# mwhoffman/pygp

Hardware: AMD Instinct MI355X
Metric: ExactGP log-lik+grad evals/sec at N=16384 D=8 SE-ARD fp64 (higher is better)
Workload: dtype f64; 1 GPU; ExactGP SE-ARD fp64 loglik+grad, N=16384 D=8 (metric config); batched-theta path: 6 independent thetas per GPU per step through gpx_loglik_batch, X/y resident in HBM; safe_mode=False, safe_mode_switches=0, launch=one process, C ABI only (no torch)

## Files before the change

### include/gpx.h

```cpp
#ifndef GPX_H
#define GPX_H

#include <stdint.h>

#ifdef __cplusplus
extern "C" {
#endif

#define GPX_VERSION 100
#define GPX_MAX_DIM 32
#define GPX_MAX_PARTS 8
#define GPX_MAX_HYPER (GPX_MAX_PARTS * (GPX_MAX_DIM + 2))

enum gpx_kind {
    GPX_SE = 1,
    GPX_MATERN1 = 2,
    GPX_MATERN3 = 3,
    GPX_MATERN5 = 4,
    GPX_PERIODIC = 5,
    GPX_SUM = 6,
    GPX_RQ = 7,
    GPX_PRODUCT = 8
};

// ... 83 lines not shown
int gpx_ep_update(gpx_t *h, const gpx_kspec *k, double mean, double tol, int max_iter,
                  double damping, int *iters, int *info);
int gpx_ep_loglik(gpx_t *h, double *lZ, double *dlZ);
int gpx_ep_posterior(gpx_t *h, const double *Xs, int64_t m, double *mu, double *s2);
int gpx_ep_posterior_full(gpx_t *h, const double *Xs, int64_t m, double *mu, double *Sigma);
int gpx_ep_get_sites(gpx_t *h, int64_t n, double *tau, double *nu, double *mu, double *s2);
int gpx_ep_timings(gpx_t *h, double *ms);
int gpx_exact_get_factor(gpx_t *h, int64_t n, double *R, double *a);
int gpx_loglik_batch(gpx_t *h, const gpx_kspec *k, const double *thetas,
                     int64_t B, int want_grad, double *lZ, double *dlZ,
                     int *info);
int gpx_batch_plan(gpx_t *h, int64_t B, int want_grad, int *plan);
int gpx_loglik_batch_multi(const gpx_kspec *k, const double *thetas, int64_t B,
                           const double *X, const double *y, int64_t n, int64_t d,
                           int want_grad, int ndev, double *lZ, double *dlZ, int *info);
int gpx_posterior_batch_multi(const gpx_kspec *k, const double *thetas, int64_t B,
                              const double *X, const double *y, int64_t n, int64_t d,
                              const double *Xs, int64_t m, int want_grad, int ndev, double *mu,
                              double *s2, double *dmu, double *ds2, int *info);
int gpx_multi_enable_timing(int ndev, int on);
int gpx_multi_batch_info(int ndev, int64_t B_per_dev, int want_grad, double *dense_ms,
                         int64_t *members, int *plans);
void gpx_batch_partition(int64_t B, int world, int rank, int64_t *lo, int64_t *hi);
int64_t gpx_multi_slot(int64_t B, int ndev);
int gpx_multi_comm_size(void);
int gpx_multi_pack(const double *rows, int64_t cnt, int width, int64_t slot, double *pack);
int gpx_multi_scatter(const double *gathered, int64_t B, int ndev, int width, double *out);
int gpx_posterior_batch(gpx_t *h, const gpx_kspec *k, const double *thetas, int64_t B,
                        const double *Xs, int64_t m, double *mu, double *s2, double *dmu,
                        double *ds2, int *info);

#define GPX_SPARSE_MAX_P 4096
enum gpx_sparse_method { GPX_FITC = 1, GPX_DTC = 2, GPX_VFE = 3 };
int gpx_sparse_update(gpx_t *h, const gpx_kspec *k, int method, const double *U, int64_t p,
                      double log_sn, double mean, int *info);
int gpx_sparse_append(gpx_t *h, const double *Xnew, const double *ynew, int64_t m, int *info);
int gpx_sparse_loglik(gpx_t *h, double *lZ, double *dlZ);
int gpx_sparse_posterior(gpx_t *h, const double *Xs, int64_t m, double *mu, double *s2,
                         double *dmu, double *ds2);
int gpx_sparse_posterior_full(gpx_t *h, const double *Xs, int64_t m, double *mu, double *Sigma);
int gpx_sparse_get_state(gpx_t *h, double *F1, double *F2, double *v);
int gpx_sparse_timings(gpx_t *h, double *ms);
int gpx_sparse_loglik_pseudo(gpx_t *h, double *lZ, double *dlZ, double *dU);
int gpx_sparse_pseudo_timing(gpx_t *h, double *ms);

int gpx_select_pivots(gpx_t *h, const gpx_kspec *k, const double *X, int64_t n, int64_t d,
                      int64_t p, double tol, int64_t *idx, double *piv, double *trace,
                      int64_t *count);
int gpx_select_timing(gpx_t *h, double *ms);

#define GPX_NTIMERS 11
int gpx_enable_timing(gpx_t *h, int on);
int gpx_get_timings(gpx_t *h, double *ms, int n);
int gpx_batch_timings(gpx_t *h, double *dense_ms, int64_t *members);
const char *gpx_timing_name(int i);

int gpx_la_gemm(gpx_t *h, int ta, int tb, int64_t M, int64_t N, int64_t K,
                double alpha, const double *A, int64_t lda, const double *B,
                int64_t ldb, double beta, double *C, int64_t ldc);
typedef struct gpx_gemm_ex_args {
    int64_t ta, tb, M, N, K, lda, ldb, ldc;
    double alpha, beta;
    int64_t flags, tile, waves, order, swizzle, use_lists, kshift, beta0_from;
    int64_t batch, strideA, strideB, strideC, strideC2;
    int64_t kchunk, nsplit, mstrideA, mstrideB, mstrideC;
    int64_t offA, offB, offC, offC2;
    int64_t b_is_c;
} gpx_gemm_ex_args;
int gpx_la_gemm_ex(gpx_t *h, const gpx_gemm_ex_args *a, const double *A, int64_t nA,
                   const double *B, int64_t nB, double *C, int64_t nC, double *C2,
                   int64_t nC2);
int gpx_la_potrf(gpx_t *h, const double *A, int64_t n, double *R, double *Rinv,
                 double *Ainv, int *info);
int gpx_la_gemm_bench(gpx_t *h, int ta, int tb, int64_t n, int reps, double *ms);
int gpx_la_gemm_bench_ex(gpx_t *h, int ta, int tb, int64_t n, int flags, int order,
                         int swizzle, int tile, int waves, int same_ab, int reps,
                         double *ms);
int gpx_la_gemm_bench_mnk(gpx_t *h, int ta, int tb, int64_t M, int64_t N, int64_t K, int flags,
                          double beta, int tile, int reps, double *ms);
int gpx_la_potrf_bench(gpx_t *h, int64_t n, int with_inverse, int reps,
                       double *ms);

int gpx_panel_graph_check(int T, int workers, int stream, int *ntasks);
int gpx_panel_grid_check(int nmem, int ncu, int *nspwg, int *workers);
int gpx_panel_graph_check_wide(int T, int E, int workers, int *ntasks);
int gpx_panel_graph_check_rhs(int T, int workers, int *ntasks);
int gpx_panel_graph_check_full(int T, int workers, int *ntasks);
int gpx_panel_solo_check(int T, int aug, int full, int value_only, int *ntasks);
int gpx_sweep_check(int T, int aug);
int gpx_sweep_check_lite(int T, int aug, int depth);

#ifdef __cplusplus
}
#endif
#endif
```

### pygp_amd/_lib.py

```python

import ctypes as C
import os
import threading

import numpy as np

__all__ = ['lib', 'Handle', 'default_handle', 'kspec_of', 'GpxError', 'device_count',
           'loglik_batch_multi', 'batch_partition',
           'KIND_SE', 'KIND_MATERN', 'KIND_PERIODIC', 'KIND_SUM', 'KIND_RQ', 'KIND_PRODUCT',
           'F64',
           'F32']

_HERE = os.path.dirname(os.path.abspath(__file__))
_LIBPATH = os.path.join(_HERE, 'libgpx.so')

KIND_SE = 1
KIND_MATERN = {1: 2, 3: 3, 5: 4}
KIND_PERIODIC = 5
KIND_SUM = 6
KIND_RQ = 7
KIND_PRODUCT = 8
F64, F32 = 0, 1
NTIMERS = 11

# ... 53 lines not shown
    'gpx_exact_eval': (C.c_int, [_vp, C.POINTER(_KSpec), C.c_double, C.c_double,
                                 C.c_int, _dp, _vp, _ip]),
    'gpx_exact_posterior': (C.c_int, [_vp, _vp, _i64, _vp, _vp]),
    'gpx_exact_posterior_grad': (C.c_int, [_vp, _vp, _i64, _vp, _vp, _vp, _vp]),
    'gpx_exact_posterior_full': (C.c_int, [_vp, _vp, _i64, _vp, _vp]),
    'gpx_kernel_gradx': (C.c_int, [_vp, C.POINTER(_KSpec), _vp, _i64, _vp, _i64, _i64,
                                   C.c_int, _vp]),
    'gpx_kernel_gradxy': (C.c_int, [_vp, C.POINTER(_KSpec), _vp, _i64, _vp, _i64, _i64, _vp]),
    'gpx_exact_posterior_gradient': (C.c_int, [_vp, _vp, _i64, _vp, _vp]),
    'gpx_gradobs_set_data': (C.c_int, [_vp, _vp, _i64, _vp, _vp, _i64, _vp, _i64]),
    'gpx_gradobs_update': (C.c_int, [_vp, C.POINTER(_KSpec), C.c_double, C.c_double,
                                     C.c_double, _ip]),
    'gpx_gradobs_loglik': (C.c_int, [_vp, _dp]),
    'gpx_gradobs_posterior': (C.c_int, [_vp, _vp, _i64, _vp, _vp]),
    'gpx_gradobs_posterior_full': (C.c_int, [_vp, _vp, _i64, _vp, _vp]),
    'gpx_kernel_matvec': (C.c_int, [_vp, C.POINTER(_KSpec), _vp, _i64, _i64, _vp, _i64, _vp]),
    'gpx_laplace_set_data': (C.c_int, [_vp, _vp, _i64, _i64, _vp]),
    'gpx_laplace_update': (C.c_int, [_vp, C.POINTER(_KSpec), C.c_int, C.c_double, C.c_double,
                                     C.c_int, C.c_int, _ip, _ip]),
    'gpx_laplace_loglik': (C.c_int, [_vp, _dp, _vp]),
    'gpx_laplace_posterior': (C.c_int, [_vp, _vp, _i64, _vp, _vp]),
    'gpx_laplace_posterior_full': (C.c_int, [_vp, _vp, _i64, _vp, _vp]),
    'gpx_laplace_get_mode': (C.c_int, [_vp, _i64, _vp, _vp]),
    'gpx_laplace_timings': (C.c_int, [_vp, _vp]),
    'gpx_ep_update': (C.c_int, [_vp, C.POINTER(_KSpec), C.c_double, C.c_double, C.c_int,
                                C.c_double, _ip, _ip]),
    'gpx_ep_loglik': (C.c_int, [_vp, _dp, _vp]),
    'gpx_ep_posterior': (C.c_int, [_vp, _vp, _i64, _vp, _vp]),
    'gpx_ep_posterior_full': (C.c_int, [_vp, _vp, _i64, _vp, _vp]),
    'gpx_ep_get_sites': (C.c_int, [_vp, _i64, _vp, _vp, _vp, _vp]),
    'gpx_ep_timings': (C.c_int, [_vp, _vp]),
    'gpx_mo_set_data': (C.c_int, [_vp, _vp, _i64, _vp, _i64, _i64]),
    'gpx_mo_update': (C.c_int, [_vp, C.POINTER(_KSpec), C.c_double, C.c_double, _ip]),
    'gpx_mo_loglik': (C.c_int, [_vp, _dp, _vp]),
    'gpx_mo_posterior': (C.c_int, [_vp, _vp, _i64, _vp, _vp]),
    'gpx_mo_posterior_full': (C.c_int, [_vp, _vp, _i64, _vp, _vp]),
    'gpx_icm_set_data': (C.c_int, [_vp, _vp, _i64, _i64, _vp, _vp, _i64]),
    'gpx_icm_update': (C.c_int, [_vp, C.POINTER(_KSpec), _vp, _vp, _vp, _ip]),
    'gpx_icm_loglik': (C.c_int, [_vp, _dp, _vp]),
    'gpx_icm_posterior': (C.c_int, [_vp, _vp, _vp, _i64, _vp, _vp]),
    'gpx_icm_posterior_full': (C.c_int, [_vp, _vp, _vp, _i64, _vp, _vp]),
    'gpx_exact_get_factor': (C.c_int, [_vp, _i64, _vp, _vp]),
    'gpx_sparse_update': (C.c_int, [_vp, C.POINTER(_KSpec), C.c_int, _vp, _i64, C.c_double,
                                    C.c_double, _ip]),
    'gpx_sparse_append': (C.c_int, [_vp, _vp, _vp, _i64, _ip]),
    'gpx_sparse_loglik': (C.c_int, [_vp, _vp, _vp]),
    'gpx_sparse_posterior': (C.c_int, [_vp, _vp, _i64, _vp, _vp, _vp, _vp]),
    'gpx_sparse_posterior_full': (C.c_int, [_vp, _vp, _i64, _vp, _vp]),
    'gpx_sparse_get_state': (C.c_int, [_vp, _vp, _vp, _vp]),
    'gpx_sparse_timings': (C.c_int, [_vp, _vp]),
    'gpx_sparse_loglik_pseudo': (C.c_int, [_vp, _vp, _vp, _vp]),
    'gpx_sparse_pseudo_timing': (C.c_int, [_vp, _vp]),
    'gpx_select_pivots': (C.c_int, [_vp, C.POINTER(_KSpec), _vp, _i64, _i64, _i64, C.c_double,
                                    _vp, _vp, _vp, C.POINTER(_i64)]),
    'gpx_select_timing': (C.c_int, [_vp, _vp]),
    'gpx_loglik_batch': (C.c_int, [_vp, C.POINTER(_KSpec), _vp, _i64, C.c_int,
                                   _vp, _vp, _vp]),
    'gpx_batch_plan': (C.c_int, [_vp, _i64, C.c_int, _ip]),
    'gpx_loglik_batch_multi': (C.c_int, [C.POINTER(_KSpec), _vp, _i64, _vp, _vp, _i64, _i64,
                                         C.c_int, C.c_int, _vp, _vp, _vp]),
    'gpx_posterior_batch_multi': (C.c_int, [C.POINTER(_KSpec), _vp, _i64, _vp, _vp, _i64, _i64,
                                            _vp, _i64, C.c_int, C.c_int, _vp, _vp, _vp, _vp,
                                            _vp]),
    'gpx_batch_partition': (None, [_i64, C.c_int, C.c_int, C.POINTER(_i64),
                                   C.POINTER(_i64)]),
    'gpx_multi_slot': (_i64, [_i64, C.c_int]),
    'gpx_multi_comm_size': (C.c_int, []),
    'gpx_multi_pack': (C.c_int, [_vp, _i64, C.c_int, _i64, _vp]),
    'gpx_multi_scatter': (C.c_int, [_vp, _i64, C.c_int, C.c_int, _vp]),
    'gpx_posterior_batch': (C.c_int, [_vp, C.POINTER(_KSpec), _vp, _i64, _vp, _i64, _vp,
                                      _vp, _vp, _vp, _vp]),
    'gpx_enable_timing': (C.c_int, [_vp, C.c_int]),
    'gpx_get_timings': (C.c_int, [_vp, _vp, C.c_int]),
    'gpx_batch_timings': (C.c_int, [_vp, _dp, C.POINTER(_i64)]),
    'gpx_timing_name': (C.c_char_p, [C.c_int]),
    'gpx_la_gemm': (C.c_int, [_vp, C.c_int, C.c_int, _i64, _i64, _i64,
                              C.c_double, _vp, _i64, _vp, _i64, C.c_double, _vp,
                              _i64]),
    'gpx_set_safe_mode': (C.c_int, [_vp, C.c_int]),
    'gpx_get_safe_mode': (C.c_int, [_vp, _ip]),
    'gpx_multi_enable_timing': (C.c_int, [C.c_int, C.c_int]),
    'gpx_multi_batch_info': (C.c_int, [C.c_int, _i64, C.c_int, _dp, C.POINTER(_i64), _ip]),
    'gpx_panel_grid_check': (C.c_int, [C.c_int, C.c_int, _ip, _ip]),
    'gpx_la_gemm_ex': (C.c_int, [_vp, _vp, _vp, _i64, _vp, _i64, _vp, _i64, _vp, _i64]),
    'gpx_la_potrf': (C.c_int, [_vp, _vp, _i64, _vp, _vp, _vp, _ip]),
    'gpx_la_gemm_bench': (C.c_int, [_vp, C.c_int, C.c_int, _i64, C.c_int, _dp]),
    'gpx_la_gemm_bench_ex': (C.c_int, [_vp, C.c_int, C.c_int, _i64, C.c_int, C.c_int,
                                       C.c_int, C.c_int, C.c_int, C.c_int, C.c_int,
                                       _dp]),
    'gpx_la_gemm_bench_mnk': (C.c_int, [_vp, C.c_int, C.c_int, _i64, _i64, _i64, C.c_int,
                                        C.c_double, C.c_int, C.c_int, _dp]),
    'gpx_la_potrf_bench': (C.c_int, [_vp, _i64, C.c_int, C.c_int, _dp]),
    'gpx_panel_graph_check': (C.c_int, [C.c_int, C.c_int, C.c_int, C.POINTER(C.c_int)]),
    'gpx_panel_graph_check_wide': (C.c_int, [C.c_int, C.c_int, C.c_int, C.POINTER(C.c_int)]),
    'gpx_panel_graph_check_rhs': (C.c_int, [C.c_int, C.c_int, C.POINTER(C.c_int)]),
    'gpx_panel_graph_check_full': (C.c_int, [C.c_int, C.c_int, C.POINTER(C.c_int)]),
    'gpx_panel_solo_check': (C.c_int, [C.c_int, C.c_int, C.c_int, C.c_int, C.POINTER(C.c_int)]),
    'gpx_sweep_check': (C.c_int, [C.c_int, C.c_int]),
    'gpx_sweep_check_lite': (C.c_int, [C.c_int, C.c_int, C.c_int]),
}

_lib = None
_lock = threading.RLock()


def lib():
    global _lib
    if _lib is None:
        with _lock:
            if _lib is None:
                if not os.path.exists(_LIBPATH):
                    raise GpxError(
                        'pygp_amd/libgpx.so is missing: build it with '
                        '`python -m pygp_amd.build` (there is no CPU fallback)')
                L = C.CDLL(_LIBPATH)
                for name, (res, args) in SIGNATURES.items():
                    f = getattr(L, name)
                    f.restype, f.argtypes = res, args
                _lib = L
    return _lib


def _ptr(a):
    return None if a is None else a.ctypes.data_as(_vp)


def _f64(a, ndim=None):
    a = np.ascontiguousarray(a, dtype=np.float64)
    if ndim is not None and a.ndim != ndim:
        raise ValueError('expected a %d-d array' % ndim)
    return a


def _pair(X1, X2, dtype=np.float64):
    X1 = np.ascontiguousarray(X1, dtype=dtype)
    if X1.ndim != 2:
        raise ValueError('expected a 2-d array')
    n1, d = X1.shape
    if X2 is None:
        return X1, n1, None, n1, d
    X2 = np.ascontiguousarray(X2, dtype=dtype)
    if X2.ndim != 2 or X2.shape[1] != d:
        raise ValueError('X1 and X2 have different dimensions')
    return X1, n1, X2, X2.shape[0], d


def check(code):
    if code == 0:
        return
    msg = lib().gpx_last_error().decode('utf-8', 'replace')
    if code > 0:
        raise np.linalg.LinAlgError(
            '%d-th leading minor of the array is not positive definite' % code)
    raise GpxError(msg or 'libgpx error %d' % code)


class KSpecHolder(object):

    def __init__(self, kind, iso, ndim, hyper=None, parts=()):
        self.parts = list(parts)
        self.hyper = None if hyper is None else _f64(np.atleast_1d(hyper))
        self.c = _KSpec()
        self.c.kind, self.c.iso, self.c.ndim = kind, int(bool(iso)), int(ndim)
        if self.parts:
            self.arr = (_KSpec * len(self.parts))(*[p.c for p in self.parts])
            self.c.nparts = len(self.parts)
# ... 599 lines not shown
    B, nth = thetas.shape
    if nth != spec.c.nhyper + 2:
        raise ValueError('thetas must have %d columns' % (spec.c.nhyper + 2))
    if (X is None) != (y is None):
        raise ValueError('pass both X and y, or neither')
    n = d = 0
    if X is not None:
        X, y = _f64(X, 2), _f64(y, 1)
        if X.shape[0] != y.shape[0]:
            raise ValueError('X and y disagree')
        n, d = X.shape
    lZ = np.empty(B)
    dlZ = np.empty((B, nth)) if grad else None
    info = np.zeros(B, dtype=np.int32)
    check(lib().gpx_loglik_batch_multi(spec.ref(), _ptr(thetas), B, _ptr(X), _ptr(y), n, d,
                                       int(grad), int(ndev), _ptr(lZ), _ptr(dlZ),
                                       _ptr(info)))
    return (lZ, dlZ) if grad else lZ


def posterior_batch_multi(spec, thetas, Xs, X=None, y=None, grad=False, ndev=1, token=None):
    return _multi_call(lambda X_, y_: _posterior_batch_multi(spec, thetas, Xs, X_, y_, grad, ndev),
                       X, y, token, ndev)


def _posterior_batch_multi(spec, thetas, Xs, X, y, grad, ndev):
    thetas = _f64(thetas, 2)
    B, nth = thetas.shape
    if nth != spec.c.nhyper + 2:
        raise ValueError('thetas must have %d columns' % (spec.c.nhyper + 2))
    if (X is None) != (y is None):
        raise ValueError('pass both X and y, or neither')
    Xs = _f64(Xs, 2)
    m, d = Xs.shape
    n = 0
    if X is not None:
        X, y = _f64(X, 2), _f64(y, 1)
        if X.shape[0] != y.shape[0] or X.shape[1] != d:
            raise ValueError('X, y and Xs disagree')
        n = X.shape[0]
    mu, s2 = np.empty((B, m)), np.empty((B, m))
    dmu = np.empty((B, m, d)) if grad else None
    ds2 = np.empty((B, m, d)) if grad else None
    info = np.zeros(B, dtype=np.int32)
    check(lib().gpx_posterior_batch_multi(spec.ref(), _ptr(thetas), B, _ptr(X), _ptr(y), n,
                                          d if X is not None else 0, _ptr(Xs), m, int(grad),
                                          int(ndev), _ptr(mu), _ptr(s2), _ptr(dmu), _ptr(ds2),
                                          _ptr(info)))
    return (mu, s2, dmu, ds2) if grad else (mu, s2)


def batch_partition(B, world, rank):
    lo, hi = _i64(0), _i64(0)
    lib().gpx_batch_partition(B, world, rank, C.byref(lo), C.byref(hi))
    return lo.value, hi.value


def multi_comm_size():
    return int(lib().gpx_multi_comm_size())


def multi_enable_timing(ndev, on=True):
    check(lib().gpx_multi_enable_timing(int(ndev), int(bool(on))))


def multi_batch_info(ndev, B_per_dev, grad=False):
    ms = (C.c_double * ndev)()
    mem = (_i64 * ndev)()
    plans = (C.c_int * (4 * ndev))()
    check(lib().gpx_multi_batch_info(int(ndev), int(B_per_dev), int(grad), ms, mem, plans))
    return [{'device': i, 'dense_ms': float(ms[i]), 'members': int(mem[i]),
             'arrangement': ('contexts', 'groups/panel', 'groups/lockstep', 'groups/solo')[plans[4 * i]],
             'members_per_group': int(plans[4 * i + 1]),
             'groups_in_flight': int(plans[4 * i + 2]),
             'safe_mode': bool(plans[4 * i + 3])} for i in range(ndev)]


def panel_grid_check(nmem, ncu=256):
    sp, wk = C.c_int(0), C.c_int(0)
    check(lib().gpx_panel_grid_check(int(nmem), int(ncu), C.byref(sp), C.byref(wk)))
    return sp.value, wk.value


def multi_pack(rows, slot):
    rows = np.ascontiguousarray(rows, dtype=np.float64)
    cnt, width = rows.shape
    pack = np.empty((int(slot), width))
    check(lib().gpx_multi_pack(_ptr(rows) if cnt else None, cnt, width, int(slot), _ptr(pack)))
    return pack


def multi_scatter(gathered, B, ndev, width):
    gathered = np.ascontiguousarray(gathered, dtype=np.float64)
    out = np.full((int(B), int(width)), np.nan)
    check(lib().gpx_multi_scatter(_ptr(gathered) if B else None, int(B), int(ndev), int(width),
                                  _ptr(out) if B else None))
    return out


def sweep_check(T, aug=False):
    check(lib().gpx_sweep_check(int(T), int(bool(aug))))


def panel_solo_check(T, aug=False, full=False, value_only=False):
    n = C.c_int(0)
    check(lib().gpx_panel_solo_check(int(T), int(bool(aug)), int(bool(full)), int(bool(value_only)),
                                     C.byref(n)))
    return n.value


def sweep_check_lite(T, aug=False, depth=-1):
    check(lib().gpx_sweep_check_lite(int(T), int(bool(aug)), int(depth)))


def panel_graph_check_rhs(T, workers=64):
    n = C.c_int(0)
    check(lib().gpx_panel_graph_check_rhs(int(T), int(workers), C.byref(n)))
    return n.value


def panel_graph_check_full(T, workers=64):
    n = C.c_int(0)
    check(lib().gpx_panel_graph_check_full(int(T), int(workers), C.byref(n)))
    return n.value


def panel_graph_check(T, workers=64, stream=True, extra=0):
    n = C.c_int(0)
    if extra:
        check(lib().gpx_panel_graph_check_wide(int(T), int(extra), int(workers), C.byref(n)))
    else:
        check(lib().gpx_panel_graph_check(int(T), int(workers), int(bool(stream)), C.byref(n)))
    return n.value


_default = None


def default_handle():
    global _default
    if _default is None:
        with _lock:
            if _default is None:
                _default = Handle()
    return _default
```

### pygp_amd/csrc/chol.hip

```cpp

#include "gpx_internal.h"

#define LB GPX_TILE

#include <algorithm>
#include <vector>

__global__ __launch_bounds__(256) void copy_block_kernel(const double *__restrict__ src,
                                                         double *__restrict__ dst, int ld,
                                                         int rows, int cols, long long stride)
{
    src += (long long)blockIdx.z * stride;
    dst += (long long)blockIdx.z * stride;
    const int c2 = blockIdx.x * 256 + threadIdx.x;
    if (2 * c2 >= cols) return;
    for (int r = blockIdx.y; r < rows; r += gridDim.y)
        reinterpret_cast<double2 *>(dst + (size_t)r * ld)[c2] =
            reinterpret_cast<const double2 *>(src + (size_t)r * ld)[c2];
}

static int copy_block(hipStream_t s, const double *src, double *dst, int ld, int rows,
                      int cols, int batch = 1, long long stride = 0)
{
    dim3 grid((cols / 2 + 255) / 256, rows < 1024 ? rows : 1024, batch);
// ... 415 lines not shown
    hipEvent_t *G = w.events + 2 * GPX_MAX_BLOCKS;
    hipEvent_t *TD = w.events + 3 * GPX_MAX_BLOCKS;
    bool lead = false;
    if (ahead) {
        GPX_EV(hipEventRecord(D[0], s));
        const bool wide0 = nb > 1 && wide_ok(w, bl.len(0), bl.len(1), 1);
        lead = w.lead && w.lead_rows >= (wide0 ? bl.off(2) : bl.len(0));
        GPX_EV(hipStreamWaitEvent(crit, lead ? w.lead : D[0], 0));
        GPX_EV(hipStreamWaitEvent(bulk, D[0], 0));
        if (aux != bulk) GPX_EV(hipStreamWaitEvent(aux, D[0], 0));
    }
    for (int k = 0; k < nb; ++k) {
        const int ok = bl.off(k), nk = bl.len(k);
        if (ahead && k > 0) GPX_EV(hipStreamWaitEvent(crit, D[k], 0));
        const bool wide = k + 1 < nb && wide_ok(w, nk, bl.len(k + 1), 1);
        if (wide)
            GPX_TRY(gpx_panel(crit, w, ok, nk, bl.len(k + 1), w.gate_total[0], w.gate_total[1]));
        else
            GPX_TRY(potrf_rec(crit, w, ok, nk, true));
        if (ahead) {
            GPX_EV(hipEventRecord(F[k], crit));
            GPX_EV(hipStreamWaitEvent(bulk, F[k], 0));
            if (lead && k == 0) GPX_EV(hipStreamWaitEvent(crit, D[0], 0));
        }
        if (fast && k + 1 < nb) {
            const int o1 = bl.off(k + 1), n1 = bl.len(k + 1), rest = w.np - o1;
            const size_t okk = (size_t)ok * ld + ok, ok1 = (size_t)ok * ld + o1;
            const size_t o11 = (size_t)o1 * ld + o1;
            if (!wide) {
                if (k >= 1) GPX_EV(hipStreamWaitEvent(crit, G[k - 1], 0));
                {
                    GemmArgs g = mk(w.W + okk, ld, w.Kinv + ok1, ld, w.A + ok1, ld, nk, n1, nk,
                                    1.0, 0.0, GEMM_KHI_M);
                    g.order = gpx_env().ord_r12;
                    GPX_TRY(gpx_gemm(crit, 1, 0, g));
                }
                if (k >= 1) GPX_EV(hipStreamWaitEvent(crit, TD[k - 1], 0));
                GPX_TRY(syrk_upper(crit, w.A + ok1, ld, w.A + o11, ld, n1, nk, w.Kinv + o11));
            }
            GPX_EV(hipEventRecord(D[k + 1], crit));
            if (rest > n1) {
                GemmArgs g = mk(w.W + okk, ld, w.Kinv + ok1 + n1, ld, w.A + ok1 + n1, ld, nk,
                                rest - n1, nk, 1.0, 0.0, GEMM_KHI_M);
                g.order = gpx_env().ord_r12;
                GPX_TRY(gpx_gemm(bulk, 1, 0, g));
            }
            GPX_EV(hipStreamWaitEvent(bulk, D[k + 1], 0));
            if (k + 2 < nb) {
                const int o2 = bl.off(k + 2), n2 = bl.len(k + 2), rest2 = w.np - o2;
                const size_t ok2 = (size_t)ok * ld + o2, o12 = (size_t)o1 * ld + o2,
                             o22 = (size_t)o2 * ld + o2;
                {
                    GemmArgs g = mk(w.A + ok1, ld, w.A + ok2, ld, w.Kinv + o12, ld, n1, rest2,
                                    nk, -1.0, 1.0, 0);
                    GPX_TRY(gpx_gemm(bulk, 1, 0, g));
                }
                GPX_TRY(gate_bump(bulk, w, 0));
                GPX_EV(hipEventRecord(G[k], bulk));
                GPX_TRY(syrk_upper(bulk, w.A + ok2, ld, w.A + o22, ld, n2, nk, w.Kinv + o22));
                GPX_TRY(gate_bump(bulk, w, 1));
                GPX_EV(hipEventRecord(TD[k], bulk));
                if (k + 3 < nb) {
                    const int o3 = bl.off(k + 3), rest3 = w.np - o3;
                    const size_t ok3 = (size_t)ok * ld + o3, o23 = (size_t)o2 * ld + o3,
                                 o33 = (size_t)o3 * ld + o3;
                    GemmArgs g = mk(w.A + ok2, ld, w.A + ok3, ld, w.Kinv + o23, ld, n2, rest3, nk,
                                    -1.0, 1.0, 0);
                    GPX_TRY(gpx_gemm(bulk, 1, 0, g));
                    GPX_TRY(syrk_upper(bulk, w.A + ok3, ld, w.A + o33, ld, rest3, nk,
                                       w.Kinv + o33));
                }
            }
        } else if (k + 1 < nb) {
            const int o1 = bl.off(k + 1), n1 = bl.len(k + 1), rest = w.np - o1;
            const size_t okk = (size_t)ok * ld + ok, ok1 = (size_t)ok * ld + o1;
            const int skip = wide ? n1 : 0;
            if (rest > skip) {
                GemmArgs g = mk(w.W + okk, ld, w.Kinv + ok1 + skip, ld, w.A + ok1 + skip, ld, nk,
                                rest - skip, nk, 1.0, 0.0, GEMM_KHI_M);
                g.order = gpx_env().ord_r12;
                GPX_TRY(gpx_gemm(bulk, 1, 0, g));
            }
            const size_t o11 = (size_t)o1 * ld + o1;
            if (!wide)
                GPX_TRY(syrk_upper(bulk, w.A + ok1, ld, w.A + o11, ld, n1, nk, w.Kinv + o11));
            if (ahead) GPX_EV(hipEventRecord(D[k + 1], bulk));
            if (k + 2 < nb) {
                const int o2 = bl.off(k + 2), rest2 = w.np - o2;
                const size_t ok2 = (size_t)ok * ld + o2, o12 = (size_t)o1 * ld + o2,
                             o22 = (size_t)o2 * ld + o2;
                {
                    GemmArgs g = mk(w.A + ok1, ld, w.A + ok2, ld, w.Kinv + o12, ld, n1, rest2,
                                    nk, -1.0, 1.0, 0);
                    GPX_TRY(gpx_gemm(bulk, 1, 0, g));
                }
                GPX_TRY(gate_bump(bulk, w, 0));
                GPX_TRY(syrk_upper(bulk, w.A + ok2, ld, w.A + o22, ld, rest2, nk, w.Kinv + o22));
                GPX_TRY(gate_bump(bulk, w, 1));
            }
        }
        if (mode != GPX_POTRF_R)
            GPX_TRY(inverse_column(aux, w, bl, k, mode == GPX_POTRF_KINV,
                                   defer && k == nb - 1 ? evW : nullptr,
                                   ahead && aux != bulk && k > 0 ? D[k] : nullptr,
                                   ahead && aux != bulk ? F[k] : nullptr));
    }
    if (ahead) {
        GPX_EV(hipEventRecord(evJoin, bulk));
        GPX_EV(hipStreamWaitEvent(s, evJoin, 0));
        if (aux != bulk) {
            GPX_EV(hipEventRecord(evAux, aux));
            GPX_EV(hipStreamWaitEvent(s, defer ? evW : evAux, 0));
        }
    }
    return 0;
}

int gpx_potrf_join(hipStream_t s, const DenseWs &w)
{
    if (w.defer_kinv && w.events && w.aux)
        GPX_EV(hipStreamWaitEvent(s, w.events[4 * GPX_MAX_BLOCKS + 1], 0));
    return 0;
}

hipEvent_t gpx_potrf_lead_event(const DenseWs &w)
{
    return w.events ? w.events[4 * GPX_MAX_BLOCKS + 3] : nullptr;
}

int gpx_trtri(hipStream_t s, const DenseWs &w)
{
    const BatchScope batch_scope(w);
    const Blocks bl(w.np);
    return trtri_blocks(s, w, bl, 0, bl.count);
}

int gpx_trsm_rt(hipStream_t s, const DenseWs &w, double *B, double *T, int ldb, int m,
                long long pstride)
{
    const BatchScope batch_scope(w);
    const Blocks bl(w.np);
    const int ld = w.ld;
    const int nb = w.batch > 1 ? w.batch : 1;
    auto panel = [&](GemmArgs g, bool a_panel) {
        if (nb > 1) {
            if (a_panel) g.strideA = pstride;
            g.strideB = pstride;
            g.strideC = pstride;
        }
        return g;
    };
    for (int k = 0; k < bl.count; ++k) {
        const int ok = bl.off(k), nk = bl.len(k);
        const size_t okk = (size_t)ok * ld + ok;
        double *Bk = B + (size_t)ok * ldb, *Tk = T + (size_t)ok * ldb;
        if (nk == LB) {
            GemmArgs g = mk(w.W + okk, ld, Bk, ldb, Bk, ldb, LB, m, LB, 1.0, 0.0, 0);
            g.tile = 128;
            GPX_TRY(gpx_gemm(s, 1, 0, panel(g, false)));
        } else {
            GPX_TRY(copy_block(s, Bk, Tk, ldb, nk, m, nb, pstride));
            GemmArgs g = mk(w.W + okk, ld, Tk, ldb, Bk, ldb, nk, m, nk, 1.0, 0.0, GEMM_KHI_M);
            g.order = 1;
            GPX_TRY(gpx_gemm(s, 1, 0, panel(g, false)));
        }
        const int o1 = bl.off(k + 1), rest = w.np - o1;
        if (rest > 0)
            GPX_TRY(gpx_gemm(s, 1, 0,
                             panel(mk(w.A + (size_t)ok * ld + o1, ld, Bk, ldb, B + (size_t)o1 * ldb,
                                      ldb, rest, m, nk, -1.0, 1.0, 0), false)));
    }
    return 0;
}

int gpx_lauum(hipStream_t s, const DenseWs &w)
{
    const BatchScope batch_scope(w);
    const int n = w.np, ld = w.ld;
    GemmArgs g = mk(w.W, ld, w.W, ld, w.Kinv, ld, n, n, n, 1.0, 0.0,
                    GEMM_UPPER_ONLY | GEMM_KLO_M | GEMM_KLO_N |
// ... 12 lines not shown
```

### pygp_amd/csrc/gpx_env.h

```cpp
#pragma once

#include <cstdlib>
#include <cstring>
#include <vector>

#define GPX_ENV_TABLE(X)                                                        \
        \
    X(int, nb0, "GPX_NB0", 0)                                                   \
    X(int, nb, "GPX_NB", 0)                                                     \
    X(const char *, blocks_text, "GPX_BLOCKS", nullptr)                         \
    X(int, split_last, "GPX_SPLIT_LAST", 0)                                     \
    X(int, lookahead, "GPX_LOOKAHEAD", 1)                                       \
    X(int, fastchain, "GPX_FASTCHAIN", 1)                                       \
    X(int, aux, "GPX_AUX", 1)                                                   \
    X(int, lead_build, "GPX_LEAD_BUILD", 1)                                     \
    X(int, defer_kinv, "GPX_DEFER_KINV", 1)                                     \
    X(int, invcol_early, "GPX_INVCOL_EARLY", -1)                                \
    X(int, overlap_nosplit, "GPX_OVERLAP_NOSPLIT", 1)                           \
    X(int, grad_whole, "GPX_GRAD_WHOLE", 4096)                                  \
    X(int, grad_full_w, "GPX_GRAD_FULL_W", 4096)                                \
       \
    X(int, swizzle, "GPX_SWIZZLE", 0)                                           \
    X(int, tile_lists, "GPX_TILE_LISTS", 1)                                     \
    X(int, ord_t, "GPX_ORD_T", 2)                                               \
    X(int, ord_r12, "GPX_ORD_R12", 1)                                           \
    X(int, ord_lauum, "GPX_ORD_LAUUM", 0)                                       \
    X(int, krev, "GPX_KREV", 0)                                                 \
    X(int, krev_invcol, "GPX_KREV_INVCOL", 0)                                   \
    X(int, tile_xcd, "GPX_TILE_XCD", -1)                                        \
    X(int, gemm_big, "GPX_GEMM_BIG", 0)                                         \
    X(int, gemm_small, "GPX_GEMM_SMALL", 0)                                     \
    X(int, gemm_small_below, "GPX_GEMM_SMALL_BELOW", 0)                         \
    X(int, gemm_nobalance, "GPX_GEMM_NOBALANCE", 0)                             \
    X(int, gemm_nosplit, "GPX_GEMM_NOSPLIT", 0)                                 \
    X(int, gemm_pipe, "GPX_GEMM_PIPE", 1)                                       \
    X(const char *, gemm_log, "GPX_GEMM_LOG", nullptr)                          \
    X(int, ldpad, "GPX_LDPAD", 32)                                              \
    X(int, bench_ldpad, "GPX_BENCH_LDPAD", 0)                                   \
                                           \
    X(int, panel, "GPX_PANEL", -1)                                              \
    X(int, panel_stream, "GPX_PANEL_STREAM", 1)                                 \
    X(int, panel_serial, "GPX_PANEL_SERIAL", 1)                                 \
    X(int, panel_strict, "GPX_PANEL_STRICT", 0)                                 \
    X(int, panel_debug, "GPX_PANEL_DEBUG", 0)                                   \
    X(int, panel_timeout_ms, "GPX_PANEL_TIMEOUT_MS", 2000)                      \
    X(int, panel_timeout_us, "GPX_PANEL_TIMEOUT_US", 0)                         \
    X(int, panel_wg, "GPX_PANEL_WG", -1)                                        \
    X(int, panel_wg_wide, "GPX_PANEL_WG_WIDE", -1)                              \
    X(int, panel_wg_whole, "GPX_PANEL_WG_WHOLE", -1)                            \
    X(int, panel_nspine, "GPX_PANEL_NSPINE", -1)                                \
    X(int, panel_mspine, "GPX_PANEL_MSPINE", -1)                                \
    X(int, panel_mwg, "GPX_PANEL_MWG", -1)                                      \
    X(int, panel_split, "GPX_PANEL_SPLIT", 1)                                   \
    X(int, panel_fold, "GPX_PANEL_FOLD", 1)                                     \
    X(int, panel_kbatch, "GPX_PANEL_KBATCH", -1)                                \
    X(int, panel_i128, "GPX_PANEL_I128", -1)                                    \
    X(int, panel_u128, "GPX_PANEL_U128", 6)                                     \
    X(double, panel_chain_scale, "GPX_PANEL_CHAIN_SCALE", 0.75)                 \
    X(int, panel_whole, "GPX_PANEL_WHOLE", GPX_PANEL_WHOLE_DEFAULT)             \
    X(int, panel_rhs, "GPX_PANEL_RHS", 1)                                       \
    X(int, panel_wide, "GPX_PANEL_WIDE", 0)                                     \
    X(int, panel_leaf_skip, "GPX_PANEL_LEAF_SKIP", 0)                           \
    X(int, leaf_skip, "GPX_LEAF_SKIP", 0)                                       \
    X(int, leaf_mfma, "GPX_LEAF_MFMA", 1)                                       \
     \
    X(int, group_max_np, "GPX_GROUP_MAX_NP", 32768)                             \
    X(int, group_members, "GPX_GROUP_MEMBERS", 0)                               \
    X(int, group_inflight, "GPX_GROUP_INFLIGHT", 0)                             \
    X(int, group_min_big, "GPX_GROUP_MIN_BIG", 2)                               \
    X(int, sweep_min_members, "GPX_SWEEP_MIN_MEMBERS", 16)                      \
    X(int, sweep_lite, "GPX_SWEEP_LITE", 1)                                     \
    X(int, sweep_fold, "GPX_SWEEP_FOLD", -1)                                    \
    X(int, sweep_pre, "GPX_SWEEP_PRE", 1)                                       \
    X(int, sweep_right, "GPX_SWEEP_RIGHT", 4)                                   \
    X(int, sweep_invblock, "GPX_SWEEP_INVBLOCK", 4)                             \
    X(int, sweep_narrow, "GPX_SWEEP_NARROW", 1)                                 \
    X(int, sweep_rhs_dense, "GPX_SWEEP_RHS_DENSE", 1)                           \
    X(int, solo_max_np, "GPX_SOLO_MAX_NP", 0)                                   \
    X(int, solo_min_members, "GPX_SOLO_MIN_MEMBERS", 16)                        \
    X(int, xs_debug, "GPX_XS_DEBUG", 0)                                         \
     \
    X(int, batch_inflight, "GPX_BATCH_INFLIGHT", 3)                             \
    X(int, batch_lookahead, "GPX_BATCH_LOOKAHEAD", -1)                          \
    X(int, twin_probe, "GPX_TWIN_PROBE", 1)                                     \
    X(int, twin_own_bulk, "GPX_TWIN_OWN_BULK", 1)                               \
    X(bool, twin_log, "GPX_TWIN_LOG", false)                                    \
    X(bool, destroy_log, "GPX_DESTROY_LOG", false)                              \
    X(int, multi_fake, "GPX_MULTI_FAKE", 0)                                     \
    X(int, multi_force_rccl, "GPX_MULTI_FORCE_RCCL", 0)                         \
                                          \
    X(int, kbuild_w, "GPX_KBUILD_W", 0)                                         \
    X(int, trace_rows, "GPX_TRACE_ROWS", 16)                                    \
                                                                \
    X(const char *, test_jitter_text, "GPX_TEST_JITTER", nullptr)               \
    X(int, test_hold_build_us, "GPX_TEST_HOLD_BUILD_US", 0)

struct GpxEnv {
#define GPX_ENV_FIELD(type, field, name, dflt) type field;
    GPX_ENV_TABLE(GPX_ENV_FIELD)
#undef GPX_ENV_FIELD
    std::vector<int> blocks;
// ... 54 lines not shown
```

### pygp_amd/csrc/panel.hip

```cpp

#include "panel_dev.h"
#include "panel_graph.h"

#include <algorithm>
#include <cstdio>
#include <cstring>
#include <unistd.h>
#include <map>
#include <mutex>
#include <tuple>
#include <vector>

struct PanelArgs {
    double *bA, *bW, *bX;
    int ld;
    const PTask *tasks;
    const PTask *spine;
    int ntasks, nspine, nspwg, nctr;
    int nmem;
    long long mstride;
    int pstride;
    const int *gates;
    int gate_need0, gate_need1;
    int *ctl;
// ... 685 lines not shown
                            tr[32 * i + 6] ? (tr[32 * i + 6] - base) * 0.01 : 0.0,
                            tr[32 * i + 7] ? (tr[32 * i + 7] - base) * 0.01 : 0.0);
                {
                    double cyc = 0.0, ticks = 0.0;
                    for (int i = 0; i < nall; ++i) {
                        cyc += (double)(tr[32 * i + 13] - tr[32 * i + 12]);
                        ticks += (double)(tr[32 * i + 2] - tr[32 * i + 1]);
                    }
                    fprintf(stderr, "  in-kernel clock %.0f MHz\n", cyc / ticks * 100.0);
                }
                for (int i = 0; i < nall; ++i)
                    if (tr[32 * i + 16]) {
                        fprintf(stderr, "  leaf %4d", i);
                        for (int q = 16; q < 31; ++q)
                            fprintf(stderr, " %.2f", tr[32 * i + q] ? (tr[32 * i + q] - base) * 0.01 : 0.0);
                        fprintf(stderr, "\n");
                    }
                for (int i = 0; i < nall; ++i)
                    if (tr[32 * i + 8])
                        fprintf(stderr, "  sub %4d %.2f %.2f %.2f %.2f\n", i,
                                (tr[32 * i + 8] - base) * 0.01, (tr[32 * i + 9] - base) * 0.01,
                                (tr[32 * i + 10] - base) * 0.01, (tr[32 * i + 11] - base) * 0.01);
            }
            return 0;
        }
        usleep(1000);
    }
    fprintf(stderr, "panel stalled: T=%d tasks=%d grid=%d\n", T, pl.ntasks, grid);
    for (int g = 0; g < grid; ++g)
        fprintf(stderr, "  wg %2d task %4d state %d dep %d need %d\n", g, dbg_host[8 * g],
                dbg_host[8 * g + 1], dbg_host[8 * g + 2], dbg_host[8 * g + 3]);
    fflush(stderr);
    _exit(3);
    return 0;
}

static int device_cus(int *out)
{
    static int ncu_of[64] = {};
    int device = 0;
    GPX_HIP(hipGetDevice(&device));
    int ncu = 256;
    if (device >= 0 && device < 64) {
        if (!ncu_of[device]) {
            hipDeviceProp_t prop;
            GPX_HIP(hipGetDeviceProperties(&prop, device));
            ncu_of[device] = prop.multiProcessorCount > 0 ? prop.multiProcessorCount : 256;
        }
        ncu = ncu_of[device];
    }
    *out = ncu;
    return 0;
}

int gpx_panel(hipStream_t s, const DenseWs &w, int off, int n, int extra, int gate_need0,
              int gate_need1, bool rhs)
{
    const int T = n / 128, E = extra / 128;
    const bool whole = n > GPX_PANEL_MAX;
    const bool aug = (whole || rhs) && extra == 128;
    if (rhs && !aug) {
        gpx_set_error("panel: a right-hand side is one tile column");
        return -1;
    }
    if (n % 128 || T < 2 || n > GPX_PANEL_WHOLE_MAX || (whole && ((extra != 0 && !aug) || off != 0)) ||
        (rhs && off != 0) ||
        !w.pctl || extra % 128 || extra < 0 || extra > GPX_PANEL_MAX ||
        (aug ? (n != w.np || w.ld < n + 128) : off + n + extra > w.np)) {
        gpx_set_error("panel: bad block (order %d, %d more columns)", n, extra);
        return -1;
    }
    GPX_TRY(gpx_test_jitter(s));
    const int nmem = w.batch > 1 ? w.batch : 1;
    if (nmem > 1 && E > 0 && !aug) {
        gpx_set_error("panel: wide panels are not member-batched");
        return -1;
    }
    const bool split = panel_split(gpx_panel_streaming(), E, aug);
    const bool solo = nmem > 1 && off == 0 && n == w.np && (E == 0 || aug) && gpx_panel_solo(w);
    int nspwg = 1, workers = 0;
    if (!solo) {
        int ncu = 0;
        GPX_TRY(device_cus(&ncu));
        if (!(nmem > 1 ? panel_grid_members(nmem, ncu, &nspwg, &workers)
                       : panel_grid_single(w.np, T, E, whole, split, ncu, &nspwg, &workers))) {
            gpx_set_error("panel: %d members need %d spine workgroups, the device has %d CUs "
                          "(run such groups through the lock-step sweep)", nmem, nmem, ncu);
            return -1;
        }
    }
    const int sched_workers = nmem > 1 ? std::min(128, std::max(4, workers / nmem)) : workers;
    PanelList pl;
    const int ig = gpx_inverse_group(w.full_w, off, n, w.np);
    GPX_TRY(panel_list(T, E, sched_workers, aug, ig, &pl, solo ? (w.no_inverse ? 2 : 1) : 0));
    const size_t o = (size_t)off * w.ld + off;
    PanelArgs p;
    p.bA = w.A + o;
    p.bW = w.W + o;
    p.bX = w.Kinv + o;
    p.ld = w.ld;
    p.tasks = pl.dev;
    p.spine = pl.dev + pl.ntasks;
    p.ntasks = pl.ntasks;
    p.nspine = pl.nspine;
    p.nspwg = std::min(nspwg, pl.nspine);
    p.nctr = pl.nctr;
    p.nmem = nmem;
    p.mstride = nmem > 1 ? w.mstride : 0;
    p.pstride = nmem > 1 ? w.pstride : 0;
    if (nmem > 1 && (w.pstride < PCTL_HEAD + pl.nctr || w.mstride <= 0)) {
        gpx_set_error("panel: bad member strides (%lld, %d)", w.mstride, w.pstride);
        return -1;
    }
    p.gates = w.pctl + PCTL_GATES;
    p.gate_need0 = gate_need0;
    p.gate_need1 = gate_need1;
    p.ctl = w.pctl;
    p.info = w.info;
    p.goff = off;
    const Handoff ho = panel_handoff(true);
    p.timeout = ho.timeout;
    p.strict = ho.strict;
    p.leafskip = ho.leafskip | (solo && w.no_inverse ? 8 : 0);
    p.dbg = nullptr;
    p.trace = nullptr;
    const int debug = gpx_env().panel_debug;
    static int *dbg_host = nullptr;
    static long long *trace_dev = nullptr;
    const int grid = (int)std::min<long long>(workers, (long long)pl.ntasks * nmem) + p.nspwg * nmem;
    if (debug && (nmem == 1 || solo)) {
        if (!dbg_host) GPX_HIP(hipHostMalloc((void **)&dbg_host, 264 * 8 * sizeof(int)));
        memset(dbg_host, 0xff, 264 * 8 * sizeof(int));
        p.dbg = dbg_host;
        if (debug >= 2 && pl.ntasks + pl.nspine <= 32768) {
            if (!trace_dev) GPX_HIP(hipMalloc((void **)&trace_dev, 32768 * 32 * sizeof(long long)));
            GPX_HIP(hipMemsetAsync(trace_dev, 0, 32768 * 32 * sizeof(long long), s));
            p.trace = trace_dev;
        }
    }
    if (gpx_panel_streaming() && T >= 2) {
        const int TWl = T + E;
        hipLaunchKernelGGL(panel_sentinel_kernel, dim3(TWl * TWl, nmem, 4), dim3(256), 0, s, p.bA,
                           p.bX, T, TWl, split ? 1 : 0, p.ld, p.mstride);
        GPX_HIP(hipGetLastError());
    }
    {
        const int serial = gpx_env().panel_serial;
        struct Last { hipEvent_t ev = nullptr; hipStream_t stream = nullptr; };
        static Last last[64];
        static std::mutex mu;
        int device = 0;
        GPX_HIP(hipGetDevice(&device));
        if (serial && !solo && device >= 0 && device < 64) {
            std::lock_guard<std::mutex> lock(mu);
            Last &l = last[device];
            if (!l.ev) GPX_HIP(hipEventCreateWithFlags(&l.ev, hipEventDisableTiming));
            if (l.stream && l.stream != s) GPX_HIP(hipStreamWaitEvent(s, l.ev, 0));
            hipLaunchKernelGGL(panel_kernel, dim3(grid), dim3(256), LEAF2_LDS, s, p);
            GPX_HIP(hipGetLastError());
            GPX_HIP(hipEventRecord(l.ev, s));
            l.stream = s;
        } else {
            hipLaunchKernelGGL(panel_kernel, dim3(grid), dim3(256), LEAF2_LDS, s, p);
            GPX_HIP(hipGetLastError());
        }
    }
    if (debug && (nmem == 1 || solo))
// ... 4 lines not shown
```

### pygp_amd/csrc/panel_graph.h

```cpp
#pragma once

#include "panel_task.h"

#include <vector>

struct GraphSpec {
    int T, E;
    bool stream;
    bool aug;
    int ig;
    bool sweep;
};

struct PanelTasks {
    std::vector<PTask> tasks;
    int ntasks = 0, nspine = 0, nctr = 0;
};
int panel_tasks(const GraphSpec &spec, int workers, int solo, PanelTasks *out);

struct SweepTasks {
    std::vector<PTask> tasks;
    std::vector<int> first, count;
};
int sweep_tasks(int T, int E, SweepTasks *out);

int panel_kbatch(int T, int E);
bool panel_split(bool stream, int E, bool aug);
bool panel_fold();

bool gpx_panel_grid_fits(int nmem, int nspwg, int ncu);
bool panel_grid_members(int nmem, int ncu, int *nspwg, int *workers);
bool panel_grid_single(int np, int T, int E, bool whole, bool split, int ncu, int *nspwg,
                       int *workers);
```

### pygp_amd/csrc/panel_graph.hip

```cpp

#include "panel_graph.h"

#include <algorithm>
#include <cstdio>
#include <cstring>
#include <queue>
#include <vector>

namespace {

struct Graph {
    const int T, ld;
    const int E;
    const bool stream;
    const int kbatch;
    const bool aug;
    const bool fold;
    const bool split;
    const int ig;
    bool ok = true;

    explicit Graph(const GraphSpec &sp)
        : T(sp.T), ld(PT_LD), E(sp.E), stream(sp.stream),
          kbatch(sp.sweep ? 1 : panel_kbatch(sp.T, sp.E)), aug(sp.aug),
// ... 418 lines not shown

int panel_kbatch(int T, int E)
{
    const int kb = gpx_env().panel_kbatch;
    if (T <= GPX_PANEL_MAX / 128 || E > 1) return 1;
    return kb > 0 ? kb : 8;
}

bool panel_split(bool stream, int E, bool aug)
{
    return gpx_env().panel_split && stream && (E == 0 || aug);
}

bool panel_fold() { return gpx_env().panel_fold != 0; }

int panel_tasks(const GraphSpec &spec, int workers, int solo, PanelTasks *out)
{
    const Graph g(spec);
    if (!g.ok) return -1;
    std::vector<PTask> sorted, leaves;
    if (solo) {
        if (!g.solo_order_ok()) {
            gpx_set_error("panel: generation order is not a sequential order (T = %d)", g.T);
            return -1;
        }
        for (const PTask &t : g.tasks)
            if (solo != 2 || t.sig < g.cX(0, 0)) leaves.push_back(t);
    } else {
        const std::vector<int> order = g.schedule(workers);
        if (order.size() != g.tasks.size()) {
            gpx_set_error("panel: scheduling failed (T = %d, E = %d)", g.T, g.E);
            return -1;
        }
        sorted.reserve(order.size());
        for (int id : order) (pt_on_spine(g.tasks[id]) ? leaves : sorted).push_back(g.tasks[id]);
        std::stable_sort(leaves.begin(), leaves.end(),
                         [](const PTask &a, const PTask &b) { return a.goff < b.goff; });
    }
    out->ntasks = (int)sorted.size();
    out->nspine = (int)leaves.size();
    out->nctr = g.nctr();
    out->tasks = std::move(sorted);
    out->tasks.insert(out->tasks.end(), leaves.begin(), leaves.end());
    return 0;
}

int sweep_tasks(int T, int E, SweepTasks *out)
{
    const Graph g({T, E, true, E == 1, PANEL_IG, true});
    if (!g.ok) return -1;
    out->tasks.clear();
    out->first.assign(T + 1, 0);
    out->count.assign(T + 1, 0);
    auto strip = [](PTask t) {
        t.ndep = 0;
        t.klo = 0;
        t.sig2 = -1;
        if (t.op == PT_XS) t.bufA = 0;
        if (t.op == PT_LEAF) t.khi = 0;
        return t;
    };
    for (int ph = 0; ph <= T; ++ph) {
        out->first[ph] = (int)out->tasks.size();
        for (int pass = 0; pass < 2; ++pass)
            for (const PTask &t : g.tasks) {
                const bool fused = PT_FUSED(t.op, t);
                if (ph == 0) {
                    if (pass == 0 && t.op == PT_LEAF && t.offA == 0) out->tasks.push_back(strip(t));
                    continue;
                }
                const int s = ph - 1;
                if (t.op != PT_XS || t.offA != g.tile(s, s) || fused != (pass == 0)) continue;
                out->tasks.push_back(strip(t));
            }
        out->count[ph] = (int)out->tasks.size() - out->first[ph];
    }
    return 0;
}

bool gpx_panel_grid_fits(int nmem, int nspwg, int ncu)
{
    return nmem >= 1 && nspwg >= 1 && (long long)nmem * nspwg + 1 <= ncu;
}
bool panel_grid_members(int nmem, int ncu, int *nspwg, int *workers)
{
    const int mspine = gpx_env().panel_mspine, mwg = gpx_env().panel_mwg;
    int sp = mspine > 0 ? mspine : (nmem <= 16 ? 3 : (nmem <= 40 ? 2 : 1));
    while (sp > 1 && !gpx_panel_grid_fits(nmem, sp, ncu)) --sp;
    if (!gpx_panel_grid_fits(nmem, sp, ncu)) return false;
    *nspwg = sp;
    *workers = std::max(8, (mwg > 0 ? mwg : 250) - nmem * sp);
    return true;
}
bool panel_grid_single(int np, int T, int E, bool whole, bool split, int ncu, int *nspwg,
                       int *workers)
{
    const GpxEnv &e = gpx_env();
    int sp = e.panel_nspine > 0 ? e.panel_nspine : (split ? (panel_fold() ? 9 : 5) : 3);
    while (sp > 1 && !gpx_panel_grid_fits(1, sp, ncu)) --sp;
    if (!gpx_panel_grid_fits(1, sp, ncu)) return false;
    *nspwg = sp;
    *workers = whole ? (e.panel_wg_whole > 0 ? e.panel_wg_whole : (T <= 16 ? 160 : 250))
               : E > 0 ? (e.panel_wg_wide > 0 ? e.panel_wg_wide : (np <= 4096 ? 96 : 64))
               : e.panel_wg > 0 ? e.panel_wg
               : np <= 4096 ? 128 : 32;
    return true;
}
extern "C" int gpx_panel_grid_check(int nmem, int ncu, int *nspwg, int *workers)
{
    if (nmem < 1 || ncu < 1) {
        gpx_set_error("panel grid check: bad arguments");
        return -1;
    }
    int sp = 0, wk = 0;
    if (!panel_grid_members(nmem, ncu, &sp, &wk)) {
        gpx_set_error("panel grid check: %d members do not fit %d CUs", nmem, ncu);
        return -1;
    }
    if (nspwg) *nspwg = sp;
    if (workers) *workers = wk;
    return 0;
}
static int panel_graph_check(int T, int E, int workers, int stream, int *ntasks, bool aug,
                             bool full_w)
{
    if (T < 2 || T > PCTL_TMAX || workers < 1 || E < 0 || E > GPX_PANEL_MAX / 128 ||
        (E > 0 && !stream) || (T > GPX_PANEL_MAX / 128 && (!stream || E > 1))) {
        gpx_set_error("panel graph check: bad arguments");
        return -1;
    }
    const Graph g({T, E, stream != 0, aug, gpx_inverse_group(full_w, 0, 128 * T, 128 * T), false});
    if (!g.ok) return -1;
    const int n = (int)g.tasks.size();
    if (ntasks) *ntasks = n;
    const std::vector<int> order = g.schedule(workers);
    if ((int)order.size() != n) {
        gpx_set_error("panel graph check: schedule has %d of %d tasks", (int)order.size(), n);
        return -1;
    }
    std::vector<char> seen(n, 0);
    Replay rp(g, "panel graph check");
    const std::vector<int> &ctr = rp.ctr;
    unsigned long long last_spine = 0;
    for (int pos = 0; pos < n; ++pos) {
        const int id = order[pos];
        if (id < 0 || id >= n || seen[id]) {
            gpx_set_error("panel graph check: position %d repeats or invents task %d", pos, id);
            return -1;
        }
        seen[id] = 1;
        const PTask &t = g.tasks[id];
        GPX_TRY(rp.run(id, -1, pos));
        if (PT_HAS_LEAF(t.op, t)) {
            const int tile = (int)(t.goff / 128);
            if (tile < 0 || tile >= T || (last_spine >> tile & 1)) {
                gpx_set_error("panel graph check: spine task of tile %d twice or out of range", tile);
                return -1;
            }
            last_spine |= 1ull << tile;
        }
    }
    if (last_spine != (1ull << T) - 1) {
        gpx_set_error("panel graph check: spine tiles %#llx of %d", last_spine, T);
        return -1;
    }
    for (int s = 0; s < T + E; ++s)
        for (int t = s; t < T + E; ++t) {
            GPX_TRY(rp.ends_at(s, t, (g.aug && s >= T) ? 0 : Graph::STAGE * (s < T ? s + 1 : T)));
            if (t >= T || s / g.ig != t / g.ig) continue;
            if (t > s && (ctr[g.cX(s, t)] != Graph::STAGE * g.inv_chunks(s, t) ||
                          ctr[g.cW(s, t)] != Graph::STAGE)) {
                gpx_set_error("panel graph check: inverse tile (%d,%d) incomplete (%d, %d)", s, t,
                              ctr[g.cX(s, t)], ctr[g.cW(s, t)]);
                return -1;
            }
        }
    return 0;
}
extern "C" int gpx_panel_graph_check(int T, int workers, int stream, int *ntasks)
{
    return panel_graph_check(T, 0, workers, stream, ntasks, false, false);
}
extern "C" int gpx_panel_graph_check_rhs(int T, int workers, int *ntasks)
{
    return panel_graph_check(T, 1, workers, 1, ntasks, true, false);
}
extern "C" int gpx_panel_graph_check_full(int T, int workers, int *ntasks)
{
    return panel_graph_check(T, 1, workers, 1, ntasks, true, true);
}
extern "C" int gpx_panel_solo_check(int T, int aug, int full, int value_only, int *ntasks)
{
    if (T < 2 || T > PCTL_TMAX) {
        gpx_set_error("panel solo check: bad arguments");
        return -1;
    }
    const Graph g({T, aug ? 1 : 0, true, aug != 0,
                   gpx_inverse_group(full != 0, 0, 128 * T, 128 * T), false});
    if (!g.ok) return -1;
    if (!g.solo_order_ok()) {
        gpx_set_error("panel solo check: generation order is not sequential (T = %d)", T);
        return -1;
    }
    Replay rp(g, "panel solo check");
// ... 141 lines not shown
```

Before: 15.47 evals/s.

## Scale spine workgroups by group size and run single trailing SYRK for large N

```diff
diff --git a/include/gpx.h b/include/gpx.h
--- a/include/gpx.h
+++ b/include/gpx.h
@@ -189,6 +189,8 @@
                        double *ms);
 
 int gpx_panel_graph_check(int T, int workers, int stream, int *ntasks);
+int gpx_panel_grid_rule(int nmem, int ncu, int tiles, int split, int fold, int *nspwg,
+                        int *workers);
 int gpx_panel_grid_check(int nmem, int ncu, int *nspwg, int *workers);
 int gpx_panel_graph_check_wide(int T, int E, int workers, int *ntasks);
 int gpx_panel_graph_check_rhs(int T, int workers, int *ntasks);
diff --git a/pygp_amd/_lib.py b/pygp_amd/_lib.py
--- a/pygp_amd/_lib.py
+++ b/pygp_amd/_lib.py
@@ -159,6 +159,7 @@
     'gpx_multi_enable_timing': (C.c_int, [C.c_int, C.c_int]),
     'gpx_multi_batch_info': (C.c_int, [C.c_int, _i64, C.c_int, _dp, C.POINTER(_i64), _ip]),
     'gpx_panel_grid_check': (C.c_int, [C.c_int, C.c_int, _ip, _ip]),
+    'gpx_panel_grid_rule': (C.c_int, [C.c_int, C.c_int, C.c_int, C.c_int, C.c_int, _ip, _ip]),
     'gpx_la_gemm_ex': (C.c_int, [_vp, _vp, _vp, _i64, _vp, _i64, _vp, _i64, _vp, _i64]),
     'gpx_la_potrf': (C.c_int, [_vp, _vp, _i64, _vp, _vp, _vp, _ip]),
     'gpx_la_gemm_bench': (C.c_int, [_vp, C.c_int, C.c_int, _i64, C.c_int, _dp]),
@@ -924,6 +925,13 @@
     return sp.value, wk.value
 
 
+def panel_grid_rule(nmem, ncu=256, tiles=8, split=True, fold=True):
+    sp, wk = C.c_int(0), C.c_int(0)
+    check(lib().gpx_panel_grid_rule(int(nmem), int(ncu), int(tiles), int(split), int(fold),
+                                    C.byref(sp), C.byref(wk)))
+    return sp.value, wk.value
+
+
 def multi_pack(rows, slot):
     rows = np.ascontiguousarray(rows, dtype=np.float64)
     cnt, width = rows.shape
diff --git a/pygp_amd/csrc/chol.hip b/pygp_amd/csrc/chol.hip
--- a/pygp_amd/csrc/chol.hip
+++ b/pygp_amd/csrc/chol.hip
@@ -521,20 +521,25 @@
                 GPX_TRY(gpx_gemm(bulk, 1, 0, g));
             }
             const size_t o11 = (size_t)o1 * ld + o1;
-            if (!wide)
+            const bool one = !ahead && !wide && w.np > 8192 && gpx_env().trail_one;
+            if (one)
+                GPX_TRY(syrk_upper(bulk, w.A + ok1, ld, w.A + o11, ld, rest, nk, w.Kinv + o11));
+            else if (!wide)
                 GPX_TRY(syrk_upper(bulk, w.A + ok1, ld, w.A + o11, ld, n1, nk, w.Kinv + o11));
             if (ahead) GPX_EV(hipEventRecord(D[k + 1], bulk));
             if (k + 2 < nb) {
                 const int o2 = bl.off(k + 2), rest2 = w.np - o2;
                 const size_t ok2 = (size_t)ok * ld + o2, o12 = (size_t)o1 * ld + o2,
                              o22 = (size_t)o2 * ld + o2;
-                {
+                if (!one) {
                     GemmArgs g = mk(w.A + ok1, ld, w.A + ok2, ld, w.Kinv + o12, ld, n1, rest2,
                                     nk, -1.0, 1.0, 0);
                     GPX_TRY(gpx_gemm(bulk, 1, 0, g));
                 }
                 GPX_TRY(gate_bump(bulk, w, 0));
-                GPX_TRY(syrk_upper(bulk, w.A + ok2, ld, w.A + o22, ld, rest2, nk, w.Kinv + o22));
+                if (!one)
+                    GPX_TRY(syrk_upper(bulk, w.A + ok2, ld, w.A + o22, ld, rest2, nk,
+                                       w.Kinv + o22));
                 GPX_TRY(gate_bump(bulk, w, 1));
             }
         }
diff --git a/pygp_amd/csrc/gpx_env.h b/pygp_amd/csrc/gpx_env.h
--- a/pygp_amd/csrc/gpx_env.h
+++ b/pygp_amd/csrc/gpx_env.h
@@ -17,6 +17,7 @@
     X(int, defer_kinv, "GPX_DEFER_KINV", 1)                                     \
     X(int, invcol_early, "GPX_INVCOL_EARLY", -1)                                \
     X(int, overlap_nosplit, "GPX_OVERLAP_NOSPLIT", 1)                           \
+    X(int, trail_one, "GPX_TRAIL_ONE", 1)                                       \
     X(int, grad_whole, "GPX_GRAD_WHOLE", 4096)                                  \
     X(int, grad_full_w, "GPX_GRAD_FULL_W", 4096)                                \
        \
diff --git a/pygp_amd/csrc/panel.hip b/pygp_amd/csrc/panel.hip
--- a/pygp_amd/csrc/panel.hip
+++ b/pygp_amd/csrc/panel.hip
@@ -791,7 +791,8 @@
     if (!solo) {
         int ncu = 0;
         GPX_TRY(device_cus(&ncu));
-        if (!(nmem > 1 ? panel_grid_members(nmem, ncu, &nspwg, &workers)
+        if (!(nmem > 1 ? panel_grid_members(nmem, ncu, whole, split, panel_fold(), &nspwg,
+                                            &workers)
                        : panel_grid_single(w.np, T, E, whole, split, ncu, &nspwg, &workers))) {
             gpx_set_error("panel: %d members need %d spine workgroups, the device has %d CUs "
                           "(run such groups through the lock-step sweep)", nmem, nmem, ncu);
diff --git a/pygp_amd/csrc/panel_graph.h b/pygp_amd/csrc/panel_graph.h
--- a/pygp_amd/csrc/panel_graph.h
+++ b/pygp_amd/csrc/panel_graph.h
@@ -29,6 +29,7 @@
 bool panel_fold();
 
 bool gpx_panel_grid_fits(int nmem, int nspwg, int ncu);
-bool panel_grid_members(int nmem, int ncu, int *nspwg, int *workers);
+bool panel_grid_members(int nmem, int ncu, bool whole, bool split, bool fold, int *nspwg,
+                        int *workers);
 bool panel_grid_single(int np, int T, int E, bool whole, bool split, int ncu, int *nspwg,
                        int *workers);
diff --git a/pygp_amd/csrc/panel_graph.hip b/pygp_amd/csrc/panel_graph.hip
--- a/pygp_amd/csrc/panel_graph.hip
+++ b/pygp_amd/csrc/panel_graph.hip
@@ -524,10 +524,15 @@
 {
     return nmem >= 1 && nspwg >= 1 && (long long)nmem * nspwg + 1 <= ncu;
 }
-bool panel_grid_members(int nmem, int ncu, int *nspwg, int *workers)
+static int graph_spines(bool split, bool fold) { return split ? (fold ? 9 : 5) : 3; }
+bool panel_grid_members(int nmem, int ncu, bool whole, bool split, bool fold, int *nspwg,
+                        int *workers)
 {
     const int mspine = gpx_env().panel_mspine, mwg = gpx_env().panel_mwg;
-    int sp = mspine > 0 ? mspine : (nmem <= 16 ? 3 : (nmem <= 40 ? 2 : 1));
+    const int least = nmem <= 16 ? 3 : (nmem <= 40 ? 2 : 1);
+    const int share = whole ? 20 : 40;
+    int sp = std::max(least, std::min(graph_spines(split, fold), share / std::max(1, nmem)));
+    if (mspine > 0) sp = mspine;
     while (sp > 1 && !gpx_panel_grid_fits(nmem, sp, ncu)) --sp;
     if (!gpx_panel_grid_fits(nmem, sp, ncu)) return false;
     *nspwg = sp;
@@ -538,7 +543,7 @@
                        int *workers)
 {
     const GpxEnv &e = gpx_env();
-    int sp = e.panel_nspine > 0 ? e.panel_nspine : (split ? (panel_fold() ? 9 : 5) : 3);
+    int sp = e.panel_nspine > 0 ? e.panel_nspine : graph_spines(split, panel_fold());
     while (sp > 1 && !gpx_panel_grid_fits(1, sp, ncu)) --sp;
     if (!gpx_panel_grid_fits(1, sp, ncu)) return false;
     *nspwg = sp;
@@ -548,20 +553,26 @@
                : np <= 4096 ? 128 : 32;
     return true;
 }
-extern "C" int gpx_panel_grid_check(int nmem, int ncu, int *nspwg, int *workers)
-{
-    if (nmem < 1 || ncu < 1) {
+extern "C" int gpx_panel_grid_rule(int nmem, int ncu, int tiles, int split, int fold, int *nspwg,
+                                   int *workers)
+{
+    if (nmem < 1 || ncu < 1 || tiles < 2 || tiles > PCTL_TMAX) {
         gpx_set_error("panel grid check: bad arguments");
         return -1;
     }
     int sp = 0, wk = 0;
-    if (!panel_grid_members(nmem, ncu, &sp, &wk)) {
+    if (!panel_grid_members(nmem, ncu, tiles > GPX_PANEL_MAX / 128, split != 0, split && fold, &sp,
+                            &wk)) {
         gpx_set_error("panel grid check: %d members do not fit %d CUs", nmem, ncu);
         return -1;
     }
     if (nspwg) *nspwg = sp;
     if (workers) *workers = wk;
     return 0;
+}
+extern "C" int gpx_panel_grid_check(int nmem, int ncu, int *nspwg, int *workers)
+{
+    return gpx_panel_grid_rule(nmem, ncu, GPX_PANEL_MAX / 128, 0, 0, nspwg, workers);
 }
 static int panel_graph_check(int T, int E, int workers, int stream, int *ntasks, bool aug,
                              bool full_w)
```

Result: faster. 15.67 evals/s (median of 6 runs) (+1.3%).
